# infraheads/tvidz

Hardware: AMD Instinct MI355X
Metric: 1080p frames/sec scene-cut scoring (luma SAD + select), frames resident in HBM (higher is better)
Workload: dtype u8

## Files before the change

tvidz_amd/csrc/tvz_scene.hip:

```cpp
#include <algorithm>

#include "tvz_common.h"

namespace {

constexpr int kWave = 64;
#ifndef TVZ_SCENE_BLOCK
#define TVZ_SCENE_BLOCK 256
#endif
constexpr int kBlock = TVZ_SCENE_BLOCK;
constexpr int kWavesPerBlock = kBlock / kWave;

struct Tuning {
    int U = 0;
    int tc = 0;
    int nt = 1;
};

struct StateHdr {
    double prev_mafd;
    int32_t have_prev;
    int32_t parity;
    int64_t frames_seen;
};
constexpr size_t kStateHdrBytes = 256;
struct WsHdr {
    double last_mafd;
};
constexpr size_t kWsHdrBytes = 256;

struct StateArgs {
    StateHdr *hdr;
    uint8_t *buf0, *buf1;
};

struct Carry {
    const uint8_t *prev0;
    uint8_t *tail;
    int32_t t_first;
};
__device__ __forceinline__ Carry read_carry(const StateArgs &sa) {
    Carry c{nullptr, nullptr, 1};
    if (sa.hdr) {
        const int32_t have = sa.hdr->have_prev, par = sa.hdr->parity;
        c.prev0 = par ? sa.buf1 : sa.buf0;
        c.tail = par ? sa.buf0 : sa.buf1;
        c.t_first = have ? 0 : 1;
    }
    return c;
}

template <int CTRL, int ROW_MASK>
__device__ __forceinline__ uint32_t dpp_add(uint32_t v) {
    return v + (uint32_t)__builtin_amdgcn_update_dpp(0, (int)v, CTRL, ROW_MASK, 0xf, false);
}

__device__ __forceinline__ uint32_t wave_sum_u32(uint32_t v) {
    v = dpp_add<0x111, 0xf>(v);
    v = dpp_add<0x112, 0xf>(v);
    v = dpp_add<0x114, 0xf>(v);
    v = dpp_add<0x118, 0xf>(v);
    v = dpp_add<0x142, 0xa>(v);
    v = dpp_add<0x143, 0xc>(v);
    return (uint32_t)__builtin_amdgcn_readlane((int)v, 63);
}

template <bool S16>
__device__ __forceinline__ uint32_t sad_dword(uint32_t a, uint32_t b, uint32_t acc) {
    if constexpr (S16) return __builtin_amdgcn_sad_u16(a, b, acc);
    else return __builtin_amdgcn_sad_u8(a, b, acc);
}

template <bool S16>
__device__ __forceinline__ uint32_t sad16(const uint4 &a, const uint4 &b, uint32_t acc) {
    acc = sad_dword<S16>(a.x, b.x, acc);
    acc = sad_dword<S16>(a.y, b.y, acc);
    acc = sad_dword<S16>(a.z, b.z, acc);
    acc = sad_dword<S16>(a.w, b.w, acc);
    return acc;
}

struct Stash {
    uint32_t v = 0;
    __device__ __forceinline__ void put(int lane, int64_t t, uint32_t total) {
        if (lane == (int)(t & 63)) v = total;
    }
    __device__ __forceinline__ void maybe_flush(int lane, int64_t t, int64_t t_lo, int64_t t_last,
                                                uint32_t *__restrict__ row) {
        if ((t & 63) == 63 || t == t_last) {
            const int64_t tb = t & ~(int64_t)63;
            const int64_t lt = tb + lane;
            if (lt >= t_lo && lt <= t) row[lt] = v;
        }
    }
};

template <bool NT>
__device__ __forceinline__ uint4 load16(const uint4 *p) {
    if constexpr (NT) {
        using v4 = __attribute__((ext_vector_type(4))) unsigned int;
        const v4 v = __builtin_nontemporal_load(reinterpret_cast<const v4 *>(p));
        return make_uint4(v.x, v.y, v.z, v.w);
    } else {
        return *p;
    }
}

template <int U, bool NT, bool S16>
__global__ __launch_bounds__(kBlock) void luma_sad_flat_kernel(
    const uint8_t *__restrict__ luma, StateArgs sa, int64_t T, int64_t frame_stride, int64_t n16,
    int32_t n_strips, int32_t tc, uint32_t *__restrict__ partial, int64_t Tpad) {
    const int lane = threadIdx.x & 63;
    const int strip = blockIdx.x * kWavesPerBlock + (threadIdx.x >> 6);
    if (strip >= n_strips) return;
    const Carry cy = read_carry(sa);
    int64_t t0 = (int64_t)blockIdx.y * tc;
    const int64_t t1 = (t0 + tc < T) ? t0 + tc : T;
    if (t0 < cy.t_first) t0 = cy.t_first;
    const bool keep_tail = cy.tail != nullptr && t1 == T;

    int64_t idx[U];
    bool ok[U];
#pragma unroll
    for (int u = 0; u < U; ++u) {
        const int64_t i = ((int64_t)strip * U + u) * kWave + lane;
        ok[u] = i < n16;
        idx[u] = ok[u] ? i : 0;
    }
    uint4 prev[U], cur[U], nxt[U];
    if (t0 >= t1) {
        if (keep_tail) {
            const uint4 *pl = reinterpret_cast<const uint4 *>(luma + (T - 1) * frame_stride);
            uint4 *pt = reinterpret_cast<uint4 *>(cy.tail);
#pragma unroll
            for (int u = 0; u < U; ++u)
                if (ok[u]) pt[idx[u]] = load16<NT>(pl + idx[u]);
        }
        return;
    }
    const uint4 *pp = (t0 == 0) ? reinterpret_cast<const uint4 *>(cy.prev0)
                                : reinterpret_cast<const uint4 *>(luma + (t0 - 1) * frame_stride);
    const uint4 *pc = reinterpret_cast<const uint4 *>(luma + t0 * frame_stride);
#pragma unroll
    for (int u = 0; u < U; ++u) prev[u] = load16<NT>(pp + idx[u]);
#pragma unroll
    for (int u = 0; u < U; ++u) cur[u] = load16<NT>(pc + idx[u]);

    uint32_t *row = partial + (int64_t)strip * Tpad;
    Stash stash;
    auto score = [&](int64_t t) {
        uint32_t acc = 0;
#pragma unroll
        for (int u = 0; u < U; ++u) {
            const uint32_t a = sad16<S16>(cur[u], prev[u], acc);
            acc = ok[u] ? a : acc;
        }
        const uint32_t total = wave_sum_u32(acc);
        stash.put(lane, t, total);
        stash.maybe_flush(lane, t, t0, t1 - 1, row);
    };
    for (int64_t t = t0; t < t1 - 1; ++t) {
        const uint4 *pn = reinterpret_cast<const uint4 *>(luma + (t + 1) * frame_stride);
#pragma unroll
        for (int u = 0; u < U; ++u) nxt[u] = load16<NT>(pn + idx[u]);
        score(t);
#pragma unroll
        for (int u = 0; u < U; ++u) {
            prev[u] = cur[u];
            cur[u] = nxt[u];
        }
    }
    score(t1 - 1);
    if (keep_tail) {
        uint4 *pt = reinterpret_cast<uint4 *>(cy.tail);
#pragma unroll
        for (int u = 0; u < U; ++u)
            if (ok[u]) pt[idx[u]] = cur[u];
    }
}

__device__ __forceinline__ uint32_t load_granule(const uint8_t *p, int nb) {
    uint32_t v = 0;
    if (nb == 4) {
        __builtin_memcpy(&v, p, 4);
    } else {
        for (int i = 0; i < nb; ++i) v |= (uint32_t)p[i] << (8 * i);
    }
    return v;
}

__device__ __forceinline__ void store_granule(uint8_t *p, uint32_t v, int nb) {
    if (nb == 4) {
        __builtin_memcpy(p, &v, 4);
    } else {
        for (int i = 0; i < nb; ++i) p[i] = (uint8_t)(v >> (8 * i));
    }
}

template <int U, bool S16>
__global__ __launch_bounds__(kBlock) void luma_sad_generic_kernel(
    const uint8_t *__restrict__ luma, StateArgs sa, int64_t T, int64_t frame_stride,
    int64_t row_stride, int32_t H, int32_t W , int32_t gpr, int64_t n_gran,
    int32_t n_strips, int32_t tc, uint32_t *__restrict__ partial, int64_t Tpad) {
    const int lane = threadIdx.x & 63;
    const int strip = blockIdx.x * kWavesPerBlock + (threadIdx.x >> 6);
    if (strip >= n_strips) return;
    const Carry cy = read_carry(sa);
    int64_t t0 = (int64_t)blockIdx.y * tc;
    const int64_t t1 = (t0 + tc < T) ? t0 + tc : T;
    if (t0 < cy.t_first) t0 = cy.t_first;
    const bool keep_tail = cy.tail != nullptr && t1 == T;

    int64_t off[U], off0[U];
    int nb[U];
#pragma unroll
    for (int u = 0; u < U; ++u) {
        const int64_t g = ((int64_t)strip * U + u) * kWave + lane;
        if (g < n_gran) {
            const int64_t y = g / gpr;
            const int32_t x = (int32_t)(g - y * gpr) * 4;
            nb[u] = (W - x < 4) ? (W - x) : 4;
            off[u] = y * row_stride + x;
            off0[u] = y * (int64_t)W + x;
        } else {
            nb[u] = 0;
            off[u] = 0;
            off0[u] = 0;
        }
    }
    uint32_t prev[U], cur[U];
    if (t0 >= t1) {
        if (keep_tail) {
#pragma unroll
            for (int u = 0; u < U; ++u)
                store_granule(cy.tail + off0[u], load_granule(luma + (T - 1) * frame_stride + off[u], nb[u]), nb[u]);
        }
        return;
    }
#pragma unroll
    for (int u = 0; u < U; ++u)
        prev[u] = (t0 == 0) ? load_granule(cy.prev0 + off0[u], nb[u])
                            : load_granule(luma + (t0 - 1) * frame_stride + off[u], nb[u]);
    uint32_t *row = partial + (int64_t)strip * Tpad;
    Stash stash;
    for (int64_t t = t0; t < t1; ++t) {
        const uint8_t *pc = luma + t * frame_stride;
        uint32_t acc = 0;
#pragma unroll
        for (int u = 0; u < U; ++u) {
            cur[u] = load_granule(pc + off[u], nb[u]);
            acc = sad_dword<S16>(cur[u], prev[u], acc);
            prev[u] = cur[u];
        }
        const uint32_t total = wave_sum_u32(acc);
        stash.put(lane, t, total);
        stash.maybe_flush(lane, t, t0, t1 - 1, row);
    }
    if (keep_tail) {
#pragma unroll
        for (int u = 0; u < U; ++u) store_granule(cy.tail + off0[u], prev[u], nb[u]);
    }
}

struct SelectParams {
    double count;
    double depth_div;
    double threshold;
};

__device__ __forceinline__ double mafd_of(uint64_t sad, const SelectParams &p) {
    return (double)sad / p.count / p.depth_div;
}

__device__ __forceinline__ void scene_epilogue(uint64_t sad, bool first, double prev_mafd,
                                               const SelectParams &p, double &mafd, double &score,
                                               uint8_t &sel) {
    if (first) {
        mafd = 0.0;
        score = 0.0;
        sel = 0;
        return;
    }
    mafd = mafd_of(sad, p);
    const double diff = fabs(mafd - prev_mafd);
    const double m = (mafd > diff) ? diff : mafd;
    float f = (float)(m / 100.);
    f = (f < 0.0f) ? 0.0f : ((f > 1.0f) ? 1.0f : f);
    score = (double)f;
    sel = (score > p.threshold) ? 1 : 0;
}

constexpr int kFinT = 64;
constexpr int kFinG = 16;

__global__ __launch_bounds__(kFinT *kFinG) void scene_finalize_kernel(
    const uint32_t *__restrict__ partial, int32_t n_strips, int64_t Tpad, int64_t T,
    const StateHdr *__restrict__ st, SelectParams sp, uint64_t *__restrict__ sad_out,
    double *__restrict__ mafd_out, double *__restrict__ score_out, uint8_t *__restrict__ sel_out,
    WsHdr *__restrict__ wh) {
    __shared__ uint64_t red[kFinG][kFinT + 1];
    int32_t t_first = 1;
    double prev_mafd_in = 0.0;
    if (st && st->have_prev) {
        t_first = 0;
        prev_mafd_in = st->prev_mafd;
    }
    const int tl = threadIdx.x & (kFinT - 1);
    const int sg = threadIdx.x / kFinT;
    const int64_t bt = (int64_t)blockIdx.x * kFinT;
    const int64_t t = bt + tl;
    uint64_t acc = 0, halo = 0;
    if (t < T && t >= t_first)
        for (int s = sg; s < n_strips; s += kFinG) acc += partial[(int64_t)s * Tpad + t];
    if (tl == 0 && bt - 1 >= t_first)
        for (int s = sg; s < n_strips; s += kFinG) halo += partial[(int64_t)s * Tpad + bt - 1];
    red[sg][tl] = acc;
    if (tl == 0) red[sg][kFinT] = halo;
    __syncthreads();
    if (threadIdx.x <= kFinT) {
        uint64_t s = 0;
#pragma unroll
        for (int g = 0; g < kFinG; ++g) s += red[g][threadIdx.x];
        red[0][threadIdx.x] = s;
    }
    __syncthreads();
    if (sg == 0 && t < T) {
        const uint64_t sad = red[0][tl];
        if (sad_out) sad_out[t] = sad;
        const bool first = t < t_first;
        double prev_mafd = prev_mafd_in;
        if (t - 1 >= t_first) prev_mafd = mafd_of(tl ? red[0][tl - 1] : red[0][kFinT], sp);
        double mafd, score;
        uint8_t sel;
        scene_epilogue(sad, first, prev_mafd, sp, mafd, score, sel);
        if (mafd_out) mafd_out[t] = mafd;
        if (score_out) score_out[t] = score;
        if (sel_out) sel_out[t] = sel;
        if (t == T - 1) wh->last_mafd = mafd;
    }
}

__global__ __launch_bounds__(256) void scene_select_kernel(const uint64_t *__restrict__ sad,
                                                           int64_t T,
                                                           const double *__restrict__ d_prev_mafd,
                                                           SelectParams sp,
                                                           uint8_t *__restrict__ sel_out,
                                                           double *__restrict__ score_out,
                                                           double *__restrict__ mafd_out) {
    const int64_t t = (int64_t)blockIdx.x * blockDim.x + threadIdx.x;
    if (t >= T) return;
    const int64_t t_first = d_prev_mafd ? 0 : 1;
    double prev_mafd = d_prev_mafd ? *d_prev_mafd : 0.0;
    if (t - 1 >= t_first) prev_mafd = mafd_of(sad[t - 1], sp);
    double mafd, score;
    uint8_t sel;
    scene_epilogue(sad[t], t < t_first, prev_mafd, sp, mafd, score, sel);
    sel_out[t] = sel;
    if (score_out) score_out[t] = score;
    if (mafd_out) mafd_out[t] = mafd;
}

constexpr int kTailBlock = 1024;
__global__ __launch_bounds__(kTailBlock) void scene_tail_kernel(
    const uint8_t *__restrict__ sel, int64_t T, int32_t *__restrict__ cuts, int32_t cuts_cap,
    StateHdr *__restrict__ st, const WsHdr *__restrict__ wh) {
    __shared__ int32_t wsum[kTailBlock / 64];
    const int lane = threadIdx.x & 63, wave = threadIdx.x >> 6;
    if (cuts) {
        const int64_t c = (T + kTailBlock - 1) / kTailBlock;
        const int64_t t0 = (int64_t)threadIdx.x * c;
        const int64_t t1 = t0 + c < T ? t0 + c : T;
        int mine = 0;
        for (int64_t t = t0; t < t1; ++t) mine += sel[t] != 0;
        int incl = mine;
#pragma unroll
        for (int off = 1; off < 64; off <<= 1) {
            const int v = __shfl_up(incl, off);
            if (lane >= off) incl += v;
        }
        if (lane == 63) wsum[wave] = incl;
        __syncthreads();
        int base = 0, total = 0;
        for (int w = 0; w < kTailBlock / 64; ++w) {
            const int v = wsum[w];
            if (w < wave) base += v;
            total += v;
        }
        int pos = base + incl - mine;
        for (int64_t t = t0; t < t1; ++t)
            if (sel[t] != 0) {
                if (pos < cuts_cap) cuts[1 + pos] = (int32_t)t;
                ++pos;
            }
        if (threadIdx.x == 0) cuts[0] = total;
    }
    if (st && threadIdx.x == 0) {
        st->prev_mafd = wh->last_mafd;
        st->have_prev = 1;
        st->parity ^= 1;
        st->frames_seen += T;
    }
}

__global__ void scene_state_reset_kernel(StateHdr *st) {
    st->prev_mafd = 0.0;
    st->have_prev = 0;
    st->parity = 0;
    st->frames_seen = 0;
}

struct Plan {
    bool flat;
    int U;
    int tc;
    int64_t n16;
    int64_t n_gran;
    int32_t gpr;
    int32_t n_strips;
    int64_t Tpad;
};

constexpr int kGenericU = 8;

bool flat_ok(const void *p, int64_t fs, int64_t rs, int32_t H, int32_t W, int bps) {
    return rs == (int64_t)W * bps && ((int64_t)H * W * bps) % 16 == 0 && fs % 16 == 0 &&
           (reinterpret_cast<uintptr_t>(p) % 16) == 0;
}

void auto_shape(int64_t T, int64_t n16, int &U, int &tc) {
    U = 8;
    const int64_t strips = tvz::ceil_div(n16, (int64_t)kWave * U);
    const int64_t chunks = std::max<int64_t>(1, 1024 / std::max<int64_t>(1, strips));
    const int64_t want = tvz::ceil_div(T, chunks);
    tc = 8;
    while (tc < 256 && tc < want) tc *= 2;
}

int decode_shape(uint32_t shape, Tuning &tn) {
    tn = Tuning{};
    if (shape == TVZ_SHAPE_AUTO) return TVZ_OK;
    tn.nt = (shape & TVZ_SHAPE_NO_NT) ? 0 : 1;
    tn.U = (int)(shape & 0xffu);
    tn.tc = (int)((shape >> 8) & 0xfffffu);
    TVZ_REQUIRE(tn.U == 0 || tn.U == 1 || tn.U == 2 || tn.U == 4 || tn.U == 8,
                "shape: U must be 0 (auto), 1, 2, 4 or 8");
    TVZ_REQUIRE(tn.tc == 0 || tn.tc == 8 || tn.tc == 16 || tn.tc == 32 || tn.tc % 64 == 0,
                "shape: tc must be 0 (auto), 8, 16, 32 or a multiple of 64");
    return TVZ_OK;
}

Plan make_plan(bool flat, int64_t T, int32_t H, int32_t W, int bps, const Tuning &tn) {
    Plan p{};
    p.flat = flat;
    p.tc = tn.tc ? tn.tc : 128;
    p.Tpad = tvz::round_up(T > 0 ? T : 1, 64);
    if (flat) {
        p.n16 = (int64_t)H * W * bps / 16;
        int aU = 4, atc = 128;
        auto_shape(T > 0 ? T : 1, p.n16, aU, atc);
        p.U = tn.U ? tn.U : aU;
        p.tc = tn.tc ? tn.tc : atc;
        p.n_strips = (int32_t)tvz::ceil_div(p.n16, (int64_t)kWave * p.U);
    } else {
        p.U = kGenericU;
        p.gpr = (W * bps + 3) / 4;
        p.n_gran = (int64_t)H * p.gpr;
        p.n_strips = (int32_t)tvz::ceil_div(p.n_gran, (int64_t)kWave * p.U);
    }
    return p;
}

size_t plan_bytes(const Plan &p) { return (size_t)p.n_strips * (size_t)p.Tpad * sizeof(uint32_t); }

int check_dims(int64_t T, int32_t H, int32_t W) {
    TVZ_REQUIRE(T >= 0, "T must be >= 0 (got %lld)", (long long)T);
    TVZ_REQUIRE(H > 0 && W > 0, "H and W must be positive (got %d x %d)", H, W);
    if ((int64_t)H * W > (int64_t)1 << 31)
        return tvz::fail(TVZ_ERR_UNSUPPORTED, "frame of %d x %d exceeds 2^31 pixels", H, W);
    return TVZ_OK;
}

size_t state_frame_bytes(int32_t H, int32_t W, int bps) {
    return (size_t)tvz::round_up((int64_t)H * W * bps, 256);
}

int launch_sad(const uint8_t *d_luma, const StateArgs &sa, int64_t T, int32_t H, int32_t W,
               int64_t fs, int64_t rs, const Plan &p, uint32_t *partial, int bps, int nt,
               hipStream_t st) {
    dim3 grid((unsigned)tvz::ceil_div(p.n_strips, kWavesPerBlock), (unsigned)tvz::ceil_div(T, p.tc));
    if (grid.y > 65535u)
        return tvz::fail(TVZ_ERR_UNSUPPORTED, "batch of %lld frames needs more than 65535 time chunks",
                         (long long)T);
    if (p.flat) {
#define TVZ_FLAT_(UU, NTV, S16V)                                                               \
    hipLaunchKernelGGL((luma_sad_flat_kernel<UU, NTV, S16V>), grid, dim3(kBlock), 0, st, d_luma,   \
                       sa, T, fs, p.n16, p.n_strips, p.tc, partial, p.Tpad)
#define TVZ_FLAT(UU)                                                                           \
    do {                                                                                       \
        if (bps == 2) { if (nt) TVZ_FLAT_(UU, true, true); else TVZ_FLAT_(UU, false, true); }   \
        else          { if (nt) TVZ_FLAT_(UU, true, false); else TVZ_FLAT_(UU, false, false); } \
    } while (0)
        switch (p.U) {
            case 1: TVZ_FLAT(1); break;
            case 2: TVZ_FLAT(2); break;
            case 4: TVZ_FLAT(4); break;
            case 8: TVZ_FLAT(8); break;
            default: return tvz::fail(TVZ_ERR_INVALID, "unsupported U=%d", p.U);
        }
#undef TVZ_FLAT
#undef TVZ_FLAT_
    } else {
        if (bps == 2)
            hipLaunchKernelGGL((luma_sad_generic_kernel<kGenericU, true>), grid, dim3(kBlock), 0, st,
                               d_luma, sa, T, fs, rs, H, W * 2, p.gpr, p.n_gran, p.n_strips,
                               p.tc, partial, p.Tpad);
        else
            hipLaunchKernelGGL((luma_sad_generic_kernel<kGenericU, false>), grid, dim3(kBlock), 0, st,
                               d_luma, sa, T, fs, rs, H, W, p.gpr, p.n_gran, p.n_strips, p.tc,
                               partial, p.Tpad);
    }
    TVZ_HIP(hipGetLastError());
    return TVZ_OK;
}

SelectParams make_sp(int32_t H, int32_t W, int32_t bitdepth, double thr) {
    SelectParams sp;
    sp.count = (double)((uint64_t)W * (uint64_t)H);
    sp.depth_div = (double)(1ULL << (bitdepth - 8));
    sp.threshold = thr;
    return sp;
}

}

TVZ_EXPORT size_t tvz_scene_workspace_bytes(int64_t T, int32_t H, int32_t W) {
    if (T < 0 || H <= 0 || W <= 0) return 0;
    const size_t a = (size_t)tvz::ceil_div((int64_t)H * W * 2 / 16 + 1, kWave) * (size_t)tvz::round_up(T > 0 ? T : 1, 64) * sizeof(uint32_t);
    const size_t b = plan_bytes(make_plan(false, T, H, W, 2, Tuning{}));
    return (a > b ? a : b) + kWsHdrBytes + 256;
}

TVZ_EXPORT size_t tvz_scene_state_bytes(int32_t H, int32_t W, int32_t bytes_per_sample) {
    if (H <= 0 || W <= 0 || (bytes_per_sample != 1 && bytes_per_sample != 2)) return 0;
    return kStateHdrBytes + 2 * state_frame_bytes(H, W, bytes_per_sample);
}

TVZ_EXPORT int tvz_scene_state_reset(void *d_state, void *hip_stream) {
    TVZ_REQUIRE(d_state != nullptr, "d_state is NULL");
    TVZ_REQUIRE(reinterpret_cast<uintptr_t>(d_state) % 256 == 0, "d_state must be 256-byte aligned");
    hipLaunchKernelGGL(scene_state_reset_kernel, dim3(1), dim3(1), 0,
                       reinterpret_cast<hipStream_t>(hip_stream), reinterpret_cast<StateHdr *>(d_state));
    TVZ_HIP(hipGetLastError());
    return TVZ_OK;
}

namespace {
int scene_scores_impl(const uint8_t *d_luma, int bps, int64_t T, int32_t H, int32_t W,
                      int64_t frame_stride_bytes, int64_t row_stride_bytes, void *d_state,
                      int32_t bitdepth, double threshold, uint64_t *d_sad_out, double *d_mafd,
                      double *d_score, uint8_t *d_selected, int32_t *d_cuts, int32_t cuts_cap,
                      void *d_workspace, size_t workspace_bytes, uint32_t shape, void *hip_stream) {
    if (int rc = check_dims(T, H, W)) return rc;
    if (T == 0) return TVZ_OK;
    TVZ_REQUIRE(d_luma != nullptr, "d_luma is NULL");
    TVZ_REQUIRE(row_stride_bytes >= (int64_t)W * bps, "row stride %lld < %d bytes",
                (long long)row_stride_bytes, W * bps);
    TVZ_REQUIRE(frame_stride_bytes >= (int64_t)(H - 1) * row_stride_bytes + (int64_t)W * bps || T == 1,
                "frame stride %lld smaller than a plane", (long long)frame_stride_bytes);
    if (bps == 1) TVZ_REQUIRE(bitdepth == 8, "8-bit entry point called with bitdepth=%d", bitdepth);
    else {
        TVZ_REQUIRE(bitdepth > 8 && bitdepth <= 16, "16-bit entry point needs 9 <= bitdepth <= 16 (got %d)", bitdepth);
        TVZ_REQUIRE(row_stride_bytes % 2 == 0 && frame_stride_bytes % 2 == 0 &&
                        reinterpret_cast<uintptr_t>(d_luma) % 2 == 0,
                    "16-bit planes must be 2-byte aligned");
    }
    TVZ_REQUIRE(d_sad_out || d_selected || d_score || d_mafd || d_state,
                "nothing to compute: every output is NULL");
    TVZ_REQUIRE(d_cuts == nullptr || (d_selected != nullptr && cuts_cap >= 0),
                "d_cuts needs d_selected and cuts_cap >= 0");
    TVZ_REQUIRE(d_workspace != nullptr, "d_workspace is NULL");
    TVZ_REQUIRE(d_state == nullptr || reinterpret_cast<uintptr_t>(d_state) % 256 == 0,
                "d_state must be 256-byte aligned");
    Tuning tn;
    if (int rc = decode_shape(shape, tn)) return rc;
    hipStream_t st = reinterpret_cast<hipStream_t>(hip_stream);
    const bool flat = flat_ok(d_luma, frame_stride_bytes, row_stride_bytes, H, W, bps);
    const Plan p = make_plan(flat, T, H, W, bps, tn);
    uintptr_t ws = (reinterpret_cast<uintptr_t>(d_workspace) + 255) & ~(uintptr_t)255;
    const size_t lost = ws - reinterpret_cast<uintptr_t>(d_workspace);
    if (workspace_bytes < lost + kWsHdrBytes + plan_bytes(p))
        return tvz::fail(TVZ_ERR_WORKSPACE, "workspace of %zu bytes, need %zu", workspace_bytes,
                         lost + kWsHdrBytes + plan_bytes(p));
    WsHdr *wh = reinterpret_cast<WsHdr *>(ws);
    uint32_t *partial = reinterpret_cast<uint32_t *>(ws + kWsHdrBytes);
    StateArgs sa{nullptr, nullptr, nullptr};
    if (d_state) {
        sa.hdr = reinterpret_cast<StateHdr *>(d_state);
        sa.buf0 = reinterpret_cast<uint8_t *>(d_state) + kStateHdrBytes;
        sa.buf1 = sa.buf0 + state_frame_bytes(H, W, bps);
    }
    if (int rc = launch_sad(d_luma, sa, T, H, W, frame_stride_bytes, row_stride_bytes, p, partial,
                            bps, tn.nt, st))
        return rc;
    const SelectParams sp = make_sp(H, W, bitdepth, threshold);
    hipLaunchKernelGGL(scene_finalize_kernel, dim3((unsigned)tvz::ceil_div(T, kFinT)),
                       dim3(kFinT * kFinG), 0, st, partial, p.n_strips, p.Tpad, T, sa.hdr, sp,
                       d_sad_out, d_mafd, d_score, d_selected, wh);
    TVZ_HIP(hipGetLastError());
    if (d_cuts || d_state) {
        hipLaunchKernelGGL(scene_tail_kernel, dim3(1), dim3(kTailBlock), 0, st, d_selected, T, d_cuts,
                           cuts_cap, sa.hdr, wh);
        TVZ_HIP(hipGetLastError());
    }
    return TVZ_OK;
}
}

TVZ_EXPORT int tvz_scene_scores_u8(const uint8_t *d_luma, int64_t T, int32_t H, int32_t W,
                                   int64_t frame_stride_bytes, int64_t row_stride_bytes,
                                   void *d_state, int32_t bitdepth, double threshold,
                                   uint64_t *d_sad_out, double *d_mafd, double *d_score,
                                   uint8_t *d_selected, int32_t *d_cuts, int32_t cuts_cap,
                                   void *d_workspace, size_t workspace_bytes, uint32_t shape,
                                   void *hip_stream) {
    return scene_scores_impl(d_luma, 1, T, H, W, frame_stride_bytes, row_stride_bytes, d_state,
                             bitdepth, threshold, d_sad_out, d_mafd, d_score, d_selected, d_cuts,
                             cuts_cap, d_workspace, workspace_bytes, shape, hip_stream);
}

TVZ_EXPORT int tvz_scene_scores_u16(const uint16_t *d_luma, int64_t T, int32_t H, int32_t W,
                                    int64_t frame_stride_bytes, int64_t row_stride_bytes,
                                    void *d_state, int32_t bitdepth, double threshold,
                                    uint64_t *d_sad_out, double *d_mafd, double *d_score,
                                    uint8_t *d_selected, int32_t *d_cuts, int32_t cuts_cap,
                                    void *d_workspace, size_t workspace_bytes, uint32_t shape,
                                    void *hip_stream) {
    return scene_scores_impl(reinterpret_cast<const uint8_t *>(d_luma), 2, T, H, W,
                             frame_stride_bytes, row_stride_bytes, d_state, bitdepth, threshold,
                             d_sad_out, d_mafd, d_score, d_selected, d_cuts, cuts_cap, d_workspace,
                             workspace_bytes, shape, hip_stream);
}

TVZ_EXPORT int tvz_luma_sad_u8(const uint8_t *d_luma, int64_t T, int32_t H, int32_t W,
                               int64_t frame_stride_bytes, int64_t row_stride_bytes,
                               uint64_t *d_sad_out, void *d_workspace, size_t workspace_bytes,
                               void *hip_stream) {
    TVZ_REQUIRE(d_sad_out != nullptr || T == 0, "d_sad_out is NULL");
    return tvz_scene_scores_u8(d_luma, T, H, W, frame_stride_bytes, row_stride_bytes, nullptr, 8,
                               0.0, d_sad_out, nullptr, nullptr, nullptr, nullptr, 0, d_workspace,
                               workspace_bytes, TVZ_SHAPE_AUTO, hip_stream);
}

TVZ_EXPORT int tvz_scene_select(const uint64_t *d_sad, int64_t T, int32_t H, int32_t W,
                                int32_t bitdepth, double threshold, const double *d_prev_mafd,
                                uint8_t *d_selected, double *d_score, double *d_mafd,
                                void *hip_stream) {
    if (int rc = check_dims(T, H, W)) return rc;
    if (T == 0) return TVZ_OK;
    TVZ_REQUIRE(d_sad && d_selected, "d_sad / d_selected is NULL");
    TVZ_REQUIRE(bitdepth >= 8 && bitdepth <= 16, "bitdepth %d out of range", bitdepth);
    const SelectParams sp = make_sp(H, W, bitdepth, threshold);
    hipLaunchKernelGGL(scene_select_kernel, dim3((unsigned)tvz::ceil_div(T, 256)), dim3(256), 0,
                       reinterpret_cast<hipStream_t>(hip_stream), d_sad, T, d_prev_mafd, sp,
                       d_selected, d_score, d_mafd);
    TVZ_HIP(hipGetLastError());
    return TVZ_OK;
}
```

Before: 3.277 million.

## Balance SAD time chunks to SIMD count and order blocks chunk-fastest

New measurement: 3.395 million (median of 6 runs). 1.04x the previous value.

```diff
diff --git a/profiles/pattern_ceiling.hip b/profiles/pattern_ceiling.hip
--- /dev/null
+++ b/profiles/pattern_ceiling.hip
@@ -0,0 +1,181 @@
+#include <hip/hip_runtime.h>
+#include <algorithm>
+#include <cstdint>
+#include <cstdio>
+#include <cstdlib>
+#include <vector>
+
+constexpr int64_t kH = 1080, kW = 1920, kFrame = kH * kW, kN16 = kFrame / 16, kT = 10000;
+
+__device__ __forceinline__ uint4 ld(const uint4 *p) {
+    using v4 = __attribute__((ext_vector_type(4))) unsigned int;
+    const v4 v = __builtin_nontemporal_load(reinterpret_cast<const v4 *>(p));
+    return make_uint4(v.x, v.y, v.z, v.w);
+}
+
+template <int CTRL, int ROW_MASK>
+__device__ __forceinline__ uint32_t dpp_add(uint32_t v) {
+    return v + (uint32_t)__builtin_amdgcn_update_dpp(0, (int)v, CTRL, ROW_MASK, 0xf, false);
+}
+
+__device__ __forceinline__ uint32_t wave_sum(uint32_t v) {
+    v = dpp_add<0x111, 0xf>(v);
+    v = dpp_add<0x112, 0xf>(v);
+    v = dpp_add<0x114, 0xf>(v);
+    v = dpp_add<0x118, 0xf>(v);
+    v = dpp_add<0x142, 0xa>(v);
+    v = dpp_add<0x143, 0xc>(v);
+    return (uint32_t)__builtin_amdgcn_readlane((int)v, 63);
+}
+
+struct Shape {
+    int U, D, body, C, tc, order;
+};
+
+template <int U, int D, int BODY>
+__global__ __launch_bounds__(256) void walk(const uint8_t *__restrict__ luma, int32_t n_strips, int32_t n_groups,
+                                            int32_t C, int64_t q, int64_t r, int32_t order,
+                                            uint32_t *__restrict__ partial, int64_t Tpad) {
+    const int lane = threadIdx.x & 63;
+    const int b = blockIdx.x;
+    const int g = order ? b / C : b % n_groups;
+    const int c = order ? b % C : b / n_groups;
+    const int strip = g * 4 + (threadIdx.x >> 6);
+    if (strip >= n_strips) return;
+    int64_t t0 = c * q + std::min<int64_t>(c, r);
+    int64_t t1 = std::min<int64_t>(t0 + q + (c < r), kT);
+    if (t0 < 1) t0 = 1;
+    if (t0 >= t1) return;
+    int64_t idx[U];
+    bool ok[U];
+#pragma unroll
+    for (int u = 0; u < U; ++u) {
+        const int64_t i = ((int64_t)strip * U + u) * 64 + lane;
+        ok[u] = i < kN16;
+        idx[u] = ok[u] ? i : 0;
+    }
+    auto fr = [&](int64_t t) { return reinterpret_cast<const uint4 *>(luma + t * kFrame); };
+    uint4 w[D + 2][U];
+#pragma unroll
+    for (int k = 0; k <= D; ++k) {
+        const int64_t f = std::min<int64_t>(t0 - 1 + k, t1 - 1);
+#pragma unroll
+        for (int u = 0; u < U; ++u) w[k][u] = ld(fr(f) + idx[u]);
+    }
+    uint32_t stash = 0, x = 0;
+    uint32_t *row = partial + (int64_t)strip * Tpad;
+    auto score = [&](int64_t t) {
+        uint32_t acc = 0;
+#pragma unroll
+        for (int u = 0; u < U; ++u) {
+            if (BODY) {
+                uint32_t a = acc;
+                a = __builtin_amdgcn_sad_u8(w[1][u].x, w[0][u].x, a);
+                a = __builtin_amdgcn_sad_u8(w[1][u].y, w[0][u].y, a);
+                a = __builtin_amdgcn_sad_u8(w[1][u].z, w[0][u].z, a);
+                a = __builtin_amdgcn_sad_u8(w[1][u].w, w[0][u].w, a);
+                acc = ok[u] ? a : acc;
+            } else {
+                x ^= w[1][u].x ^ w[1][u].y ^ w[1][u].z ^ w[1][u].w;
+            }
+        }
+        if (BODY) {
+            const uint32_t tot = wave_sum(acc);
+            if (lane == (int)(t & 63)) stash = tot;
+            if ((t & 63) == 63 || t == t1 - 1) {
+                const int64_t lt = (t & ~(int64_t)63) + lane;
+                if (lt >= t0 && lt <= t) row[lt] = stash;
+            }
+        }
+    };
+    auto shift = [&]() {
+#pragma unroll
+        for (int k = 0; k <= D; ++k)
+#pragma unroll
+            for (int u = 0; u < U; ++u) w[k][u] = w[k + 1][u];
+    };
+    int64_t t = t0;
+    for (; t + D < t1; ++t) {
+#pragma unroll
+        for (int u = 0; u < U; ++u) w[D + 1][u] = ld(fr(t + D) + idx[u]);
+        score(t);
+        shift();
+    }
+    for (; t < t1; ++t) {
+        score(t);
+        shift();
+    }
+    if (!BODY && x == 0x9e3779b9u) row[0] = x;
+}
+
+template <int U, int D, int BODY>
+static void launch(const Shape &s, const uint8_t *luma, uint32_t *partial, int64_t Tpad) {
+    const int n_strips = (int)((kN16 + 64 * U - 1) / (64 * U));
+    const int n_groups = (n_strips + 3) / 4;
+    int64_t q, r;
+    int C;
+    if (s.tc) { q = s.tc; r = 0; C = (int)((kT + s.tc - 1) / s.tc); }
+    else { C = s.C; q = kT / C; r = kT % C; }
+    hipLaunchKernelGGL((walk<U, D, BODY>), dim3(n_groups * C), dim3(256), 0, 0, luma, n_strips, n_groups, C, q, r,
+                       s.order, partial, Tpad);
+}
+
+static void run(const Shape &s, const uint8_t *luma, uint32_t *partial, int64_t Tpad) {
+#define PC_(UU, DD, BB) if (s.U == UU && s.D == DD && s.body == BB) launch<UU, DD, BB>(s, luma, partial, Tpad)
+    PC_(8, 1, 0); PC_(8, 1, 1); PC_(8, 2, 0); PC_(8, 2, 1);
+    PC_(4, 1, 0); PC_(4, 1, 1); PC_(4, 2, 0); PC_(4, 2, 1); PC_(4, 3, 0); PC_(4, 3, 1);
+#undef PC_
+}
+
+int main(int argc, char **argv) {
+    const size_t bytes = (size_t)kT * kFrame;
+    const int64_t Tpad = (kT + 63) / 64 * 64;
+    uint8_t *luma;
+    uint32_t *partial;
+    if (hipMalloc(&luma, bytes) != hipSuccess) return 1;
+    if (hipMalloc(&partial, (size_t)(kN16 / 64 + 1) * Tpad * 4) != hipSuccess) return 1;
+    (void)hipMemset(luma, 7, bytes);
+    std::vector<Shape> shapes;
+    if (argc == 6) {
+        const Shape s{atoi(argv[1]), atoi(argv[2]), atoi(argv[3]), atoi(argv[4]), 0, atoi(argv[5])};
+        for (int k = 0; k < 4; ++k) run(s, luma, partial, Tpad);
+        return hipDeviceSynchronize() == hipSuccess ? 0 : 2;
+    }
+    for (int body : {0, 1}) {
+        shapes.push_back({8, 1, body, 0, 256, 0});
+        for (int C : {4, 8, 12, 16, 24, 40})
+            for (int order : {0, 1}) {
+                shapes.push_back({8, 1, body, C, 0, order});
+                shapes.push_back({8, 2, body, C, 0, order});
+            }
+        for (int C : {4, 8, 16, 32})
+            for (int D : {1, 2, 3}) shapes.push_back({4, D, body, C, 0, 0});
+    }
+    std::vector<std::vector<float>> ms(shapes.size());
+    hipEvent_t a, b;
+    (void)hipEventCreate(&a);
+    (void)hipEventCreate(&b);
+    for (int round = 0; round < 6; ++round)
+        for (size_t i = 0; i < shapes.size(); ++i) {
+            run(shapes[i], luma, partial, Tpad);
+            (void)hipEventRecord(a, 0);
+            for (int k = 0; k < 3; ++k) run(shapes[i], luma, partial, Tpad);
+            (void)hipEventRecord(b, 0);
+            if (hipEventSynchronize(b) != hipSuccess) return 2;
+            float m = 0;
+            (void)hipEventElapsedTime(&m, a, b);
+            if (round) ms[i].push_back(m / 3);
+        }
+    if (hipGetLastError() != hipSuccess) return 3;
+    const double alg = (double)(kT - 1) * kFrame;
+    for (size_t i = 0; i < shapes.size(); ++i) {
+        std::vector<float> v = ms[i];
+        std::sort(v.begin(), v.end());
+        const Shape &s = shapes[i];
+        printf("{\"body\": \"%s\", \"U\": %d, \"D\": %d, \"C\": %d, \"tc\": %d, \"order\": %d, \"median_ms\": %.4f, "
+               "\"min_ms\": %.4f, \"max_ms\": %.4f, \"TBps_median\": %.3f}\n",
+               s.body ? "sad" : "xor", s.U, s.D, s.C, s.tc, s.order, v[v.size() / 2], v.front(), v.back(),
+               alg / (v[v.size() / 2] * 1e-3) / 1e12);
+    }
+    return 0;
+}
diff --git a/profiles/scene_step_gaps.py b/profiles/scene_step_gaps.py
--- /dev/null
+++ b/profiles/scene_step_gaps.py
@@ -0,0 +1,27 @@
+#!/usr/bin/env python3
+import csv
+import json
+import statistics
+import sys
+
+NAMES = ("luma_sad_flat_kernel", "scene_finalize_kernel", "scene_tail_kernel")
+ev = []
+for r in csv.DictReader(open(sys.argv[1])):
+    k = next((n for n in NAMES if n in r["Kernel_Name"]), None)
+    if k:
+        ev.append((int(r["Start_Timestamp"]), int(r["End_Timestamp"]), k))
+ev.sort()
+dur, gap, step = {}, {}, []
+for i, (s, e, k) in enumerate(ev):
+    dur.setdefault(k, []).append((e - s) / 1e3)
+    if i + 1 < len(ev):
+        gap.setdefault(f"{k} -> {ev[i + 1][2]}", []).append((ev[i + 1][0] - e) / 1e3)
+    if k == NAMES[0] and i > 0:
+        step.append((s - prev) / 1e3)
+    if k == NAMES[0]:
+        prev = s
+med = lambda v: round(statistics.median(v), 2)
+print(json.dumps({"launches": {k: len(v) for k, v in dur.items()}, "kernel_us_median": {k: med(v) for k, v in dur.items()},
+                  "kernel_us_min_max": {k: [round(min(v), 2), round(max(v), 2)] for k, v in dur.items()},
+                  "gap_us_median": {k: med(v) for k, v in gap.items()},
+                  "sad_start_to_next_sad_start_us_median": med(step) if step else None}))
diff --git a/profiles/summarize_scene_pmc.py b/profiles/summarize_scene_pmc.py
--- /dev/null
+++ b/profiles/summarize_scene_pmc.py
@@ -0,0 +1,36 @@
+#!/usr/bin/env python3
+import collections
+import csv
+import glob
+import json
+import sys
+
+KEEP = ("luma_sad_flat_kernel", "scene_finalize_kernel", "scene_tail_kernel", "walk<")
+for arg in sys.argv[1:]:
+    label, d = arg.split("=", 1)
+    agg = collections.defaultdict(lambda: collections.defaultdict(list))
+    for f in glob.glob(f"{d}/**/*counter_collection.csv", recursive=True):
+        for r in csv.DictReader(open(f)):
+            k = r["Kernel_Name"].replace("(anonymous namespace)::", "")
+            if any(x in k for x in KEEP):
+                k = k.split("(")[0].replace("void ", "")
+                agg[k][(r["Dispatch_Id"], r["Counter_Name"])].append(float(r["Counter_Value"]))
+    for k, per in agg.items():
+        tot = collections.defaultdict(list)
+        for (disp, name), v in per.items():
+            tot[name].append(sum(v))
+        row = {"label": label, "kernel": k}
+        for name, v in sorted(tot.items()):
+            row[name] = sum(v) / len(v)
+        if "FETCH_SIZE" in row:
+            row["read_GB_x2"] = row["FETCH_SIZE"] * 1024 * 2 / 1e9
+        if "SQ_WAVE_CYCLES" in row and "SQ_WAIT_ANY" in row:
+            row["wait_any_per_wave_cycle"] = row["SQ_WAIT_ANY"] / row["SQ_WAVE_CYCLES"]
+        if "SQ_WAVE_CYCLES" in row and "SQ_INST_LEVEL_VMEM" in row:
+            row["vmem_in_flight_per_wave"] = row["SQ_INST_LEVEL_VMEM"] / row["SQ_WAVE_CYCLES"]
+        if "GRBM_GUI_ACTIVE" in row:
+            for n in ("TA_TA_BUSY_sum", "TD_TD_BUSY_sum"):
+                if n in row:
+                    row[n.split("_")[0] + "_busy_share"] = row[n] / row["GRBM_GUI_ACTIVE"] / 256
+        row["dispatches"] = max(len(v) for v in tot.values())
+        print(json.dumps({a: (round(b, 4) if isinstance(b, float) else b) for a, b in row.items()}))
diff --git a/tvidz_amd/csrc/tvz_scene.hip b/tvidz_amd/csrc/tvz_scene.hip
--- a/tvidz_amd/csrc/tvz_scene.hip
+++ b/tvidz_amd/csrc/tvz_scene.hip
@@ -1,4 +1,6 @@
 #include <algorithm>
+#include <atomic>
+#include <climits>
 
 #include "tvz_common.h"
 
@@ -106,16 +108,37 @@
     }
 }
 
+struct Chunk {
+    int64_t t0, t1;
+};
+__device__ __forceinline__ Chunk chunk_of(int64_t c, int64_t q, int32_t r, int64_t T) {
+    const int64_t t0 = c * q + (c < r ? c : r);
+    const int64_t t1 = t0 + q + (c < r ? 1 : 0);
+    return Chunk{t0, t1 < T ? t1 : T};
+}
+
+__device__ __forceinline__ int block_group(int32_t n_chunks, int32_t n_groups, bool chunk_fastest) {
+    const uint32_t g = chunk_fastest ? blockIdx.x / (uint32_t)n_chunks : blockIdx.x % (uint32_t)n_groups;
+    return __builtin_amdgcn_readfirstlane((int)g);
+}
+__device__ __forceinline__ int block_chunk(int32_t n_chunks, int32_t n_groups, bool chunk_fastest) {
+    const uint32_t c = chunk_fastest ? blockIdx.x % (uint32_t)n_chunks : blockIdx.x / (uint32_t)n_groups;
+    return __builtin_amdgcn_readfirstlane((int)c);
+}
+
 template <int U, bool NT, bool S16>
 __global__ __launch_bounds__(kBlock) void luma_sad_flat_kernel(
     const uint8_t *__restrict__ luma, StateArgs sa, int64_t T, int64_t frame_stride, int64_t n16,
-    int32_t n_strips, int32_t tc, uint32_t *__restrict__ partial, int64_t Tpad) {
+    int32_t n_strips, int32_t n_chunks, int64_t q, int32_t r, int32_t chunk_fastest,
+    uint32_t *__restrict__ partial, int64_t Tpad) {
+    const int32_t n_groups = (n_strips + kWavesPerBlock - 1) / kWavesPerBlock;
     const int lane = threadIdx.x & 63;
-    const int strip = blockIdx.x * kWavesPerBlock + (threadIdx.x >> 6);
+    const int strip = block_group(n_chunks, n_groups, chunk_fastest) * kWavesPerBlock + (threadIdx.x >> 6);
     if (strip >= n_strips) return;
     const Carry cy = read_carry(sa);
-    int64_t t0 = (int64_t)blockIdx.y * tc;
-    const int64_t t1 = (t0 + tc < T) ? t0 + tc : T;
+    const Chunk ch = chunk_of(block_chunk(n_chunks, n_groups, chunk_fastest), q, r, T);
+    int64_t t0 = ch.t0;
+    const int64_t t1 = ch.t1;
     if (t0 < cy.t_first) t0 = cy.t_first;
     const bool keep_tail = cy.tail != nullptr && t1 == T;
 
@@ -201,13 +224,16 @@
 __global__ __launch_bounds__(kBlock) void luma_sad_generic_kernel(
     const uint8_t *__restrict__ luma, StateArgs sa, int64_t T, int64_t frame_stride,
     int64_t row_stride, int32_t H, int32_t W , int32_t gpr, int64_t n_gran,
-    int32_t n_strips, int32_t tc, uint32_t *__restrict__ partial, int64_t Tpad) {
+    int32_t n_strips, int32_t n_chunks, int64_t q, int32_t r, int32_t chunk_fastest,
+    uint32_t *__restrict__ partial, int64_t Tpad) {
+    const int32_t n_groups = (n_strips + kWavesPerBlock - 1) / kWavesPerBlock;
     const int lane = threadIdx.x & 63;
-    const int strip = blockIdx.x * kWavesPerBlock + (threadIdx.x >> 6);
+    const int strip = block_group(n_chunks, n_groups, chunk_fastest) * kWavesPerBlock + (threadIdx.x >> 6);
     if (strip >= n_strips) return;
     const Carry cy = read_carry(sa);
-    int64_t t0 = (int64_t)blockIdx.y * tc;
-    const int64_t t1 = (t0 + tc < T) ? t0 + tc : T;
+    const Chunk ch = chunk_of(block_chunk(n_chunks, n_groups, chunk_fastest), q, r, T);
+    int64_t t0 = ch.t0;
+    const int64_t t1 = ch.t1;
     if (t0 < cy.t_first) t0 = cy.t_first;
     const bool keep_tail = cy.tail != nullptr && t1 == T;
 
@@ -412,7 +438,10 @@
 struct Plan {
     bool flat;
     int U;
-    int tc;
+    int32_t n_chunks;
+    int64_t q;
+    int32_t r;
+    int32_t chunk_fastest;
     int64_t n16;
     int64_t n_gran;
     int32_t gpr;
@@ -427,13 +456,27 @@
            (reinterpret_cast<uintptr_t>(p) % 16) == 0;
 }
 
-void auto_shape(int64_t T, int64_t n16, int &U, int &tc) {
+int simd_count() {
+    static std::atomic<int> cache[64];
+    int dev = 0;
+    if (hipGetDevice(&dev) != hipSuccess || dev < 0 || dev >= 64) return 1024;
+    int n = cache[dev].load(std::memory_order_relaxed);
+    if (n == 0) {
+        int cus = 0;
+        if (hipDeviceGetAttribute(&cus, hipDeviceAttributeMultiprocessorCount, dev) != hipSuccess || cus <= 0)
+            return 1024;
+        n = 4 * cus;
+        cache[dev].store(n, std::memory_order_relaxed);
+    }
+    return n;
+}
+
+void auto_plan(int64_t T, int64_t n16, int &U, int32_t &n_chunks) {
     U = 8;
     const int64_t strips = tvz::ceil_div(n16, (int64_t)kWave * U);
-    const int64_t chunks = std::max<int64_t>(1, 1024 / std::max<int64_t>(1, strips));
-    const int64_t want = tvz::ceil_div(T, chunks);
-    tc = 8;
-    while (tc < 256 && tc < want) tc *= 2;
+    int64_t c = std::max<int64_t>(1, simd_count() / std::max<int64_t>(1, strips));
+    c = std::min<int64_t>(c, std::max<int64_t>(1, T / 8));
+    n_chunks = (int32_t)c;
 }
 
 int decode_shape(uint32_t shape, Tuning &tn) {
@@ -452,21 +495,32 @@
 Plan make_plan(bool flat, int64_t T, int32_t H, int32_t W, int bps, const Tuning &tn) {
     Plan p{};
     p.flat = flat;
-    p.tc = tn.tc ? tn.tc : 128;
-    p.Tpad = tvz::round_up(T > 0 ? T : 1, 64);
+    const int64_t Tc = T > 0 ? T : 1;
+    p.Tpad = tvz::round_up(Tc, 64);
+    int tc = tn.tc ? tn.tc : 128;
     if (flat) {
         p.n16 = (int64_t)H * W * bps / 16;
-        int aU = 4, atc = 128;
-        auto_shape(T > 0 ? T : 1, p.n16, aU, atc);
+        int aU = 8;
+        int32_t chunks = 1;
+        auto_plan(Tc, p.n16, aU, chunks);
         p.U = tn.U ? tn.U : aU;
-        p.tc = tn.tc ? tn.tc : atc;
         p.n_strips = (int32_t)tvz::ceil_div(p.n16, (int64_t)kWave * p.U);
+        if (!tn.tc) {
+            p.n_chunks = chunks;
+            p.q = Tc / chunks;
+            p.r = (int32_t)(Tc % chunks);
+            p.chunk_fastest = 1;
+            return p;
+        }
     } else {
         p.U = kGenericU;
         p.gpr = (W * bps + 3) / 4;
         p.n_gran = (int64_t)H * p.gpr;
         p.n_strips = (int32_t)tvz::ceil_div(p.n_gran, (int64_t)kWave * p.U);
     }
+    p.q = tc;
+    p.r = 0;
+    p.n_chunks = (int32_t)std::min<int64_t>(tvz::ceil_div(Tc, (int64_t)tc), INT32_MAX);
     return p;
 }
 
@@ -487,14 +541,14 @@
 int launch_sad(const uint8_t *d_luma, const StateArgs &sa, int64_t T, int32_t H, int32_t W,
                int64_t fs, int64_t rs, const Plan &p, uint32_t *partial, int bps, int nt,
                hipStream_t st) {
-    dim3 grid((unsigned)tvz::ceil_div(p.n_strips, kWavesPerBlock), (unsigned)tvz::ceil_div(T, p.tc));
-    if (grid.y > 65535u)
-        return tvz::fail(TVZ_ERR_UNSUPPORTED, "batch of %lld frames needs more than 65535 time chunks",
-                         (long long)T);
+    const int64_t blocks = tvz::ceil_div((int64_t)p.n_strips, (int64_t)kWavesPerBlock) * p.n_chunks;
+    if (blocks > INT32_MAX)
+        return tvz::fail(TVZ_ERR_UNSUPPORTED, "batch of %lld frames needs more than 2^31 blocks", (long long)T);
+    const dim3 grid((unsigned)blocks);
     if (p.flat) {
 #define TVZ_FLAT_(UU, NTV, S16V)                                                               \
     hipLaunchKernelGGL((luma_sad_flat_kernel<UU, NTV, S16V>), grid, dim3(kBlock), 0, st, d_luma,   \
-                       sa, T, fs, p.n16, p.n_strips, p.tc, partial, p.Tpad)
+                       sa, T, fs, p.n16, p.n_strips, p.n_chunks, p.q, p.r, p.chunk_fastest, partial, p.Tpad)
 #define TVZ_FLAT(UU)                                                                           \
     do {                                                                                       \
         if (bps == 2) { if (nt) TVZ_FLAT_(UU, true, true); else TVZ_FLAT_(UU, false, true); }   \
@@ -513,11 +567,11 @@
         if (bps == 2)
             hipLaunchKernelGGL((luma_sad_generic_kernel<kGenericU, true>), grid, dim3(kBlock), 0, st,
                                d_luma, sa, T, fs, rs, H, W * 2, p.gpr, p.n_gran, p.n_strips,
-                               p.tc, partial, p.Tpad);
+                               p.n_chunks, p.q, p.r, p.chunk_fastest, partial, p.Tpad);
         else
             hipLaunchKernelGGL((luma_sad_generic_kernel<kGenericU, false>), grid, dim3(kBlock), 0, st,
-                               d_luma, sa, T, fs, rs, H, W, p.gpr, p.n_gran, p.n_strips, p.tc,
-                               partial, p.Tpad);
+                               d_luma, sa, T, fs, rs, H, W, p.gpr, p.n_gran, p.n_strips,
+                               p.n_chunks, p.q, p.r, p.chunk_fastest, partial, p.Tpad);
     }
     TVZ_HIP(hipGetLastError());
     return TVZ_OK;
```
